# Pi-Star-Lab/RESCO

Measured on AMD Instinct MI355X. Metric: env-steps/sec, higher is better.
Workload: dtype f32; 1 GPU; ingolstadt21 x 4096 lock-step envs per GPU (BASELINE config 3), fixed demand from the map's rou.xml, on-device seeded random policy, Krauss sigma 0.5 + speedFactor dev 0.1; tls_expiry=1, map=ingolstadt21, envs_per_gpu=4096, pipes=2, ticks_per_env_step=10, block_threads=512, lds_bytes_per_env=40896, parallelism=env-batch split x1, no collective on the data path

## Files before the change

### resco_amd/csrc/resco_step.h

```cpp
#pragma once
#include "resco_tables.h"

struct State {
    char *base;
    size_t nc;
    int32_t *trip_log;
    int32_t *env;
    int32_t *tls;
    long long *stats;
    uint16_t *dep_next;
    uint32_t *mail;
    RS_HD float *pos() const { return (float *)base; }
    RS_HD float *speed() const { return RS_G((float *)(base + 4 * nc)); }
    RS_HD float *accel() const { return RS_G((float *)(base + 8 * nc)); }
    RS_HD float *tloss() const { return RS_G((float *)(base + 12 * nc)); }
    RS_HD float *sf() const { return RS_G((float *)(base + 16 * nc)); }
    RS_HD uint32_t *coop(int par) const { return RS_G((uint32_t *)(base + (par ? 43 : 20) * nc)); }
    RS_HD uint32_t *cooplead(int par) const { return RS_G((uint32_t *)(base + (par ? 47 : 24) * nc)); }
    RS_HD uint16_t *lane() const { return RS_G((uint16_t *)(base + 28 * nc)); }
    RS_HD uint16_t *trip() const { return RS_G((uint16_t *)(base + 30 * nc)); }
    RS_HD uint16_t *cursor() const { return RS_G((uint16_t *)(base + 32 * nc)); }
    RS_HD uint16_t *swait() const { return RS_G((uint16_t *)(base + 34 * nc)); }
    RS_HD uint16_t *rwait() const { return RS_G((uint16_t *)(base + 36 * nc)); }
    RS_HD uint16_t *depart() const { return RS_G((uint16_t *)(base + 38 * nc)); }
// ... 100 lines not shown
    uint8_t fl;
    uint16_t sfq;
};
#define FL_H 1
#define FL_MH 2
#define FL_LC 4
#define FL_MH1 8
RS_DEV int fl_mh(int t) { return (t & 1) ? FL_MH1 : FL_MH; }
#define LCT_LEFT 16
#define LCT_RIGHT 32
#define LCT_SWAP_LEFT 64
#define LCT_SWAP_RIGHT 128
struct __attribute__((aligned(8))) Aux {
    uint16_t lane, rq, nlink;
    uint16_t swait;
};
template <class Tp> struct LPtr {
    uint32_t off;
    RS_MEM Tp &operator[](int i) const { return ((Tp *)(RS_SMEM + off))[i]; }
    RS_MEM operator Tp *() const { return (Tp *)(RS_SMEM + off); }
};
struct Lds {
    LPtr<Node> node;
    LPtr<Aux> aux;
    LPtr<float> vnx, vtp;
    LPtr<uint16_t> grid;
    uint32_t gstride;
    LPtr<int32_t> arr;
    LPtr<uint16_t> dep, dep_t;
    LPtr<uint32_t> alive, alive0, insm;
    LPtr<uint32_t> mailw;
    LPtr<int32_t> agg_q, agg_a, agg_w, agg_m, agg_n;
    LPtr<uint32_t> agg_s;
    LPtr<int32_t> sig_arr, sig_dep;
    LPtr<int32_t> phase, left, nextp;
    LPtr<uint8_t> tstate;
    LPtr<int32_t> sc;
    LPtr<uint16_t> ls_h, ls_lc, ls_mh;
    uint32_t lcap;
    float cell_inv;
};
#define SC_T 0
#define SC_NINS 1
#define SC_HW 2
#define SC_NACT 3
#define SC_HWNEW 4
#define SC_ROOM 5
#define SC_HWOUT 6
#define SC_NH 7
#define SC_NLC 8
#define SC_NMH 9
#define SC_CHUNK_P 11
#define SC_CHUNK_M 12
#define SC_STATS 13
#ifndef RS_LIST_CHUNK
#define RS_LIST_CHUNK 64
#endif
#ifndef RS_H_CHUNK
#define RS_H_CHUNK RS_LIST_CHUNK
#endif

RS_CARVE size_t align16(size_t x) { return (x + 15) & ~(size_t)15; }
RS_CARVE int lds_list_cap(int C) {
#ifdef RS_LIST_CAP
    (void)C;
    return RS_LIST_CAP;
#else
    return ((C / 4 + 63) / 64) * 64;
#endif
}
RS_CARVE size_t lds_carve(Lds *L, int C, int n_cells, int n_arr, int n_dep, int n_obs, int S, int n_vt, int tls_maxl) {
    size_t o = 0;
#define CARVE(field, bytes) { if (L) L->field.off = (uint32_t)o; o += align16(bytes); }
    CARVE(node, (size_t)C * 16) CARVE(aux, (size_t)C * 8) CARVE(vnx, (size_t)C * 4)
    CARVE(sc, (size_t)(SC_STATS + ST_N) * 4)
    CARVE(alive, (size_t)((C + 31) / 32) * 4) CARVE(alive0, (size_t)((C + 31) / 32) * 4)
    {
        const int cap = lds_list_cap(C);
        if (L) L->lcap = (uint32_t)cap;
        CARVE(ls_h, (size_t)cap * 2) CARVE(ls_lc, (size_t)cap * 2) CARVE(ls_mh, (size_t)cap * 2)
    }
    const uint32_t grid_off = (uint32_t)o;
    const size_t grid_bytes = align16((size_t)((n_cells + 8 + 7) & ~7) * 2);
    if (L) L->gstride = (uint32_t)((n_cells + 8 + 7) & ~7);
    CARVE(grid, (size_t)((n_cells + 8 + 7) & ~7) * 2)
    CARVE(insm, (size_t)((n_dep + 31) / 32) * 4)
    CARVE(mailw, (size_t)((C + 31) / 32) * 4)
    CARVE(vtp, (size_t)n_vt * VT_COLS * 4)
    CARVE(phase, (size_t)S * 4) CARVE(left, (size_t)S * 4) CARVE(nextp, (size_t)S * 4)
    CARVE(sig_arr, (size_t)S * 4) CARVE(sig_dep, (size_t)S * 4)
    CARVE(tstate, (size_t)S * tls_maxl)
    CARVE(arr, (size_t)n_arr * 4) CARVE(dep, (size_t)n_dep * 2) CARVE(dep_t, (size_t)n_dep * 2)
    {
        const size_t ab = align16((size_t)n_obs * 4);
        uint32_t p = grid_off;
        if (6 * ab > grid_bytes) {
            p = (uint32_t)(align16((size_t)C * 16) + align16((size_t)C * 8));
            if (6 * ab > align16((size_t)C * 4)) { p = (uint32_t)o; o += 6 * ab; }
        }
        if (L) {
            L->agg_q.off = p; L->agg_a.off = p + (uint32_t)ab; L->agg_w.off = p + (uint32_t)(2 * ab);
            L->agg_m.off = p + (uint32_t)(3 * ab); L->agg_s.off = p + (uint32_t)(4 * ab); L->agg_n.off = p + (uint32_t)(5 * ab);
        }
    }
#undef CARVE
    return o;
}
// ... 265 lines not shown
    return f.slot;
}

template <class LT> RS_DEV int tls_state(const KTab &T, const LT &L, int tls, int pos) {
    if (tls == 0xFF) return TLS_G;
    return L.tstate[tls * T.tls_maxl + pos];
}
RS_DEV uint16_t cache_link(const KTab &T, const LaneRec &LR, int lane, int rq, int trip) {
    if (LR.link_cnt == 0) return NLINK_NONE;
    if (LR.flags & LF_INTERNAL) { const int l = LR.link_start; return (uint16_t)(l | (T.links()[l].arr_idx >= 0 ? NLINK_ARR : 0)); }
    return T.next_link()[((size_t)rq * T.kmax + (lane - (int)LR.edge_lane0)) * 2 + (trip & 1)];
}
template <class LT> RS_DEV bool foe_blocked(const KTab &T, const LT &L, const Grid &grid, const LinkRec &K) {
    for (int i = K.foe_start; i < K.foe_start + K.foe_cnt; ++i) {
        const FoeRec F = T.foes()[i];
        if (F.tls != 0xFF && tls_state(T, L, F.tls, F.tls_pos) == TLS_R) continue;
        if (F.arr_idx >= 0 && L.arr[F.arr_idx] < RM_FOE_GAP_Q) return true;
        if (F.via1_cell0 != 0xFFFF && cells_have_mover(grid, F.via1_cell0, F.via1_nc)) return true;
        if (F.via2_cell0 != 0xFFFF && cells_have_mover(grid, F.via2_cell0, F.via2_nc)) return true;
    }
    return false;
}
template <class LT> RS_DEV void tls_refresh(const KTab &T, const LT &L, const KParams &P, int s, int ph) {
    const int w = T.tls_maxl >> 2;
    const uint32_t *src = (const uint32_t *)((P.fixed_program ? T.cold.fix8 + T.cold.fix_state_off[s] : T.cold.tls8 + T.cold.tls_state_off[s]) + ph * T.tls_maxl);
    uint32_t *dst = (uint32_t *)((uint8_t *)L.tstate + s * T.tls_maxl);
    uint32_t v[8];
#pragma unroll
    for (int i = 0; i < 8; ++i) v[i] = src[i < w ? i : 0];
#pragma unroll
    for (int i = 0; i < 8; ++i) if (i < w) dst[i] = v[i];
#pragma unroll 1
    for (int i = 8; i < w; ++i) dst[i] = src[i];
}
template <class LT> RS_DEV void set_phase(const KTab &T, const LT &L, const KParams &P, int s, int ph) {
    if (ph < 0 || ph >= T.cold.tls_nphase[s]) return;
    L.phase[s] = ph;
    L.left[s] = P.tls_expiry ? T.cold.tls_dur[T.cold.tls_dur_off[s] + ph] : RM_TLS_HOLD_TICKS;
    tls_refresh(T, L, P, s, ph);
}
template <class LT> RS_DEV void tls_begin_of_tick(const KTab &T, const LT &L, const KParams &P, int s, int tick) {
    if (P.do_fsm && !P.fixed_program && tick == T.yellow_length) set_phase(T, L, P, s, L.nextp[s]);
    int left = L.left[s];
    if (left == 0) {
        const int32_t *dur = P.fixed_program ? T.cold.fix_dur + T.cold.fix_dur_off[s] : T.cold.tls_dur + T.cold.tls_dur_off[s];
        const int Pn = P.fixed_program ? T.cold.fix_nphase[s] : T.cold.tls_nphase[s];
        const int ph = (L.phase[s] + 1) % Pn;
        left = dur[ph];
        L.phase[s] = ph;
        tls_refresh(T, L, P, s, ph);
    }
    L.left[s] = left - 1;
}
struct ContRow { float c[4]; const float *cn; };
RS_DEV ContRow cont_row(const KTab &T, int rq) {
    ContRow R;
    R.cn = T.route_cont() + (size_t)rq * T.kmax;
    for (int j = 0; j < 4; ++j) R.c[j] = j < T.kmax ? R.cn[j] : 0.0f;
    return R;
}
RS_DEV float cont_of(const ContRow &R, int j) {
    return j == 0 ? R.c[0] : (j == 1 ? R.c[1] : (j == 2 ? R.c[2] : (j == 3 ? R.c[3] : R.cn[j])));
}
#define OCC_NONE (Grid{(uint16_t *)0, 0u})
#define OCC_FULL (Grid{(uint16_t *)1, 0u})
RS_DEV bool cont_notbest(float c) { return rs_float_as_int(c) < 0; }
RS_DEV float cont_len(float c) { return rs_int_as_float(rs_float_as_int(c) & 0x7FFFFFFF); }
RS_DEV int strategic_dir(const ContRow &R, int kk, int n, float x, float v, int extra, float &rem, const Grid &grid, int cell0, int nc, float occ_unit) {
    const float mine = cont_of(R, kk);
    rem = cont_len(mine) - x;
#ifdef RS_EMU_CHECK_MAIL
    { float best = 0.0f; for (int j = 0; j < n; ++j) { const float c = cont_len(cont_of(R, j)); if (c > best) best = c; }
      for (int j = 0; j < n; ++j) RS_ASSERT(cont_notbest(cont_of(R, j)) == !(cont_len(cont_of(R, j)) >= best - RM_CONT_EPS)) }
#endif
    if (!cont_notbest(mine)) return 0;
    int dl = 1000, dr = 1000;
    for (int j = kk + 1; j < n; ++j) if (!cont_notbest(cont_of(R, j))) { dl = j - kk; break; }
    for (int j = kk - 1; j >= 0; --j) if (!cont_notbest(cont_of(R, j))) { dr = kk - j; break; }
    const int dir = (dr <= dl) ? -1 : +1;
    if (grid.c == (uint16_t *)1) return dir;
    const int off = (dr <= dl ? dr : dl) + extra;
    const float la = (v > RM_LOOK_MIN_SPEED ? v : RM_LOOK_MIN_SPEED) * RM_LOOK_TIME + RM_LOOK_BASE;
    int cnt = 0;
    if (grid.c != (uint16_t *)0) cnt = cells_count(grid, cell0 + ((dr <= dl) ? -dr : dl) * nc, nc);
    if (rem - (float)cnt * occ_unit >= la * (float)off) return 0;
    return dir;
}
RS_DEV uint32_t link_reg_word(const KTab &T, int nlk) { return ((const uint32_t *)&T.links()[nlk & 0x7FFF])[2]; }
template <class LT> RS_DEV void register_approach_w(const KTab &T, const LT &L, uint32_t kw, float v, float pos, float lane_len, int vt) {
    const int st = tls_state(T, L, (int)((kw >> 16) & 0xFFu), (int)(kw >> 24));
    if (st == TLS_R) return;
    const float dist = lane_len - pos;
    if (st == TLS_Y && dist >= d_brake_gap(v, L.vtp[vt * VT_COLS + VT_DECEL])) return;
    const float ta = RS_DIV(dist, v > 1.0f ? v : 1.0f);
    const int q = ta * 10.0f >= 65000.0f ? 65000 : (int)(ta * 10.0f);
    rs_atomic_min(&L.arr[(int16_t)(kw & 0xFFFFu)], q);
}
template <class LT> RS_DEV void register_approach(const KTab &T, const LT &L, int nlk, float v, float pos, float lane_len, int vt) {
    if (!(nlk & NLINK_ARR)) return;
    if (v <= RM_HALT_SPEED) return;
    register_approach_w(T, L, link_reg_word(T, nlk), v, pos, lane_len, vt);
}
template <class LT> RS_DEV void follow_neighbour(const KTab &T, const LT &L, uint32_t key, bool clamp_gap, const LaneRec &LR, int lane, float x, float v,
                             float b, float tau, float mingap, float &vsafe) {
    const int X = (int)(key & 0xFFFFu), kx = (int)(key >> 16);
    if ((int)L.node[X].trip != kx) return;
    const int lx = L.aux[X].lane;
    if (lx == (int)LANE_NONE || (LR.flags & LF_INTERNAL)) return;
    const int l0 = LR.edge_lane0, n = LR.flags >> 2;
    if (lx < l0 || lx >= l0 + n) return;
    const float *vo = L.vtp + L.node[X].vt * VT_COLS;
    const float px = L.node[X].pos, backx = px - vo[VT_LENGTH];
    if (clamp_gap ? !(px >= x) : !(backx >= x)) return;
    float g = backx - x - mingap;
    if (clamp_gap && g < 0.0f) g = 0.0f;
    float vs = d_follow_speed(g, L.node[X].speed, b, vo[VT_DECEL], tau);
    float vc = v - b; if (vc < 0.0f) vc = 0.0f;
    if (vs < vc) vs = vc;
    if (vs < vsafe) vsafe = vs;
    (void)lane;
}

template <class LT> RS_DEV void mail_flag_set(const LT &L, int s, int par) { rs_atomic_or((uint32_t *)((Node *)L.node + s) + 3, SFQ_MAIL(par) << 16); }
template <class LT> RS_DEV void mail_flag_clear(const LT &L, int s, int par) { rs_atomic_and((uint32_t *)((Node *)L.node + s) + 3, ~(SFQ_MAIL(par) << 16)); }
template <class LT, class LP> RS_DEV void list_push(const LT &L, const LP &list, int counter, int s);
template <class LT> RS_DEV void flag_mover(const LT &L, int s, int t, int lct = 0) {
    uint32_t *w = (uint32_t *)((Node *)L.node + s) + 3;
    const uint32_t bit = (uint32_t)fl_mh(t) << 8;
    if (!(rs_atomic_fetch_or(w, bit | ((uint32_t)lct << 8)) & bit)) list_push(L, L.ls_mh, SC_NMH + (t & 1), s);
}
template <class LT, class LP> RS_DEV void list_push(const LT &L, const LP &list, int counter, int s) {
    const int i = rs_wave_ticket(&L.sc[counter]);
    if (i < (int)L.lcap) list[i] = (uint16_t)s;
}
RS_DEV float plan_vfree(const float *vt, float v, float lane_vmax, float sf) {
    float vfree = v + vt[VT_ACCEL];
    const float vl = lane_vmax * sf;
    if (vl < vfree) vfree = vl;
    if (vt[VT_MAXSPEED] < vfree) vfree = vt[VT_MAXSPEED];
    return vfree;
}
RS_DEV float plan_look(const float *vt, float vfree) { return d_brake_gap(vfree, vt[VT_DECEL]) + vfree * vt[VT_TAU] + vt[VT_MINGAP] + 1.0f; }
RS_DEV bool looks_beyond(const float *vt, float v, float x, float lane_len, float lane_vmax, float sf) {
    return lane_len - x < plan_look(vt, plan_vfree(vt, v, lane_vmax, sf));
}
RS_DEV bool may_change_lanes_row(const ContRow &R, const LaneRec &LR, int lane, int k, float x, float v, int t) {
    const int n = LR.flags >> 2;
    if ((LR.flags & LF_INTERNAL) || n < 2) return false;
    const int kk = lane - (int)LR.edge_lane0;
    float rem;
    if (strategic_dir(R, kk, n, x, v, 0, rem, OCC_FULL, 0, 0, 0.0f) != 0) return true;
    if ((((uint32_t)t >> 1) + (uint32_t)k) & 3u) return false;
    const int tk = kk + ((t & 1) ? -1 : +1);
    return tk >= 0 && tk < n && strategic_dir(R, tk, n, x, v, RM_SG_EXTRA_LANES, rem, OCC_NONE, 0, 0, 0.0f) == 0;
}
RS_DEV bool may_change_lanes(const KTab &T, int rq, uint32_t nb, const LaneRec &LR, int lane, int k, float x, float v, int t) {
    const int n = LR.flags >> 2;
    if ((LR.flags & LF_INTERNAL) || n < 2) return false;
    const int kk = lane - (int)LR.edge_lane0;
    bool r;
    if ((nb >> kk) & 1u) r = true;
    else if ((((uint32_t)t >> 1) + (uint32_t)k) & 3u) r = false;
    else {
        const int tk = kk + ((t & 1) ? -1 : +1);
        if (tk < 0 || tk >= n) r = false;
        else if (!((nb >> tk) & 1u)) r = true;
        else { float rem; r = strategic_dir(cont_row(T, rq), tk, n, x, v, RM_SG_EXTRA_LANES, rem, OCC_NONE, 0, 0, 0.0f) == 0; }
    }
#ifdef RS_EMU_CHECK_MAIL
    RS_ASSERT(r == may_change_lanes_row(cont_row(T, rq), LR, lane, k, x, v, t))
#endif
    return r;
}
template <class LT> RS_DEV int classify(const KTab &T, const LT &L, int s, const float *vt, float v, float x, const LaneRec &LR, int lane, int rq, uint32_t nb, int k, float sf, int t) {
    int fl = 0;
    if (looks_beyond(vt, v, x, LR.len, LR.vmax, sf)) { fl |= FL_H; list_push(L, L.ls_h, SC_NH, s); }
    if (may_change_lanes(T, rq, nb, LR, lane, k, x, v, t)) { fl |= FL_LC; list_push(L, L.ls_lc, SC_NLC, s); }
    return fl;
}

template <bool LONG, class LT> RS_DEV void phase_plan(const KTab &T, const LT &L, const Grid &grid, const State &G, size_t eo, const KParams &P, int genv, int t, int s) {
    RS_SEC_BEGIN
    const Aux ax = L.aux[s];
    const int lane = ax.lane;
    if (lane == (int)LANE_NONE) return;
    const Node me = L.node[s];
    const int k = me.trip;
    const float *vt = L.vtp + me.vt * VT_COLS;
    const float a = vt[VT_ACCEL], b = vt[VT_DECEL], tau = vt[VT_TAU], mingap = vt[VT_MINGAP];
    const float v = me.speed, x = me.pos;
    const float sf = sf_of(me.sfq);
    const LaneRec LR0 = T.lanes()[lane];
    LaneRec LR = LR0;
    float vsafe = RM_BIGF;
    float tgap = 0.0f, tvl = 0.0f, tbl = b;
    bool have = false;
    if (LONG) RS_SEC(7)
    const float vfree = plan_vfree(vt, v, LR.vmax, sf);
    const float look = plan_look(vt, vfree);
    const Found ld = leader_found(L, grid, LR.cell0, lane_cells(L, LR), x, k, s, look + T.maxlen);
    const int lead = ld.slot;
    if (LONG) RS_SEC(8)
    bool found = false;
    if (lead != NIL) {
        const float *vo = L.vtp + ld.vt() * VT_COLS;
        tgap = ld.pos() - vo[VT_LENGTH] - x - mingap;
        tvl = ld.speed(); tbl = vo[VT_DECEL];
        have = true; found = true;
    }
    if (me.sfq & SFQ_MAIL((t + 1) & 1)) {
        const int q = (t + 1) & 1;
        const uint32_t c1 = G.coop(q)[eo + s], c2 = G.cooplead(q)[eo + s];
        if (c1 != COOP_NONE) { G.coop(q)[eo + s] = COOP_NONE; follow_neighbour(T, L, c1, false, LR, lane, x, v, b, tau, mingap, vsafe); }
        if (c2 != COOP_NONE) { G.cooplead(q)[eo + s] = COOP_NONE; follow_neighbour(T, L, c2, true, LR, lane, x, v, b, tau, mingap, vsafe); }
        mail_flag_clear(L, s, q);
    }
#ifdef RS_EMU_CHECK_MAIL
    else { RS_ASSERT(G.coop((t + 1) & 1)[eo + s] == COOP_NONE && G.cooplead((t + 1) & 1)[eo + s] == COOP_NONE) }
#endif
    if (LONG) RS_SEC(9)
    float seen = LR.len - x;
    RS_ASSERT(LONG || found || !(seen < look))
    if (LONG && !found && seen < look) {
        int rq = ax.rq;
        int link = (int)(ax.nlink & 0x7FFF);
        int cur_lane = lane;
        const float bgv = d_brake_gap(v, b);
        for (int hop = 0; hop < RM_MAX_HOPS; ++hop) {
            const bool cur_int = (LR.flags & LF_INTERNAL) != 0;
            if (hop > 0) link = (int)(cache_link(T, LR, cur_lane, rq, k) & 0x7FFF);
            bool stop_here = false;
            LinkRec K;
            if (link == NLINK_NONE) {
                if (!cur_int && T.rsteps()[rq].next_edge == 0xFFFF) break;
                stop_here = true;
            } else {
                K = T.links()[link];
                const int st = tls_state(T, L, K.tls, K.tls_pos);
                if (K.tls != 0xFF && (st == TLS_R || st == TLS_Y) && seen >= bgv) stop_here = true;
                if (!stop_here && !(K.flags & KF_CONT) && ((K.flags & KF_MINOR) || (K.tls != 0xFF && st == TLS_g))) {
                    if (seen > RM_VIS_DIST) stop_here = true;
                    else if (K.foe_cnt > 0 && foe_blocked(T, L, grid, K)) stop_here = true;
                }
            }
            if (stop_here) {
                const float g = seen - RM_STOP_OFFSET;
                tgap = g > 0.0f ? g : 0.0f; tvl = 0.0f; tbl = b;
                have = true;
                break;
            }
            LR = K.dest;
            cur_lane = K.to_lane;
            {
                const float vnl = LR.vmax * sf;
                if (vnl < vfree) {
                    const float vs = d_free_speed(seen, vnl, b);
                    if (vs < vsafe) vsafe = vs;
                }
            }
            const Found od = rearmost_within(L, grid, LR.cell0, lane_cells(L, LR), look - seen + T.maxlen);
            if (od.slot != NIL) {
                const float *vo = L.vtp + od.vt() * VT_COLS;
                tgap = seen + od.pos() - vo[VT_LENGTH] - mingap;
                tvl = od.speed(); tbl = vo[VT_DECEL];
                have = true;
                break;
            }
            if (!cur_int) rq += 1;
            seen += LR.len;
            if (!(seen < look)) break;
        }
    }
    if (LONG) RS_SEC(10)
    if (have) {
        const float vs = d_follow_speed(tgap, tvl, b, tbl, tau);
        if (vs < vsafe) vsafe = vs;
    }
    float vmin_n = v - b; if (vmin_n < 0.0f) vmin_n = 0.0f;
    float vmin_e = v - vt[VT_EMERGENCY]; if (vmin_e < 0.0f) vmin_e = 0.0f;
    const float lo = vsafe > vmin_e ? vsafe : vmin_e;
    const float vmin = vmin_n < lo ? vmin_n : lo;
    float vmax = vfree < vsafe ? vfree : vsafe;
    if (vmax < vmin) vmax = vmin;
    const float sigma = P.sigma >= 0.0f ? P.sigma : vt[VT_SIGMA];
    float vd = vmax;
    if (sigma > 0.0f) {
        const float r = d_u01(d_hash(P.seed, (uint32_t)genv, (uint32_t)k, (uint32_t)t, 0u));
        if (vd < a) vd -= sigma * vd * r; else vd -= sigma * a * r;
        if (vd < 0.0f) vd = 0.0f;
    }
    const float vnext = vd > vmin ? vd : vmin;
    L.vnx[s] = vnext;
#ifdef RS_EMU_DEBUG
    if (s == rs_dbg_slot && (t == rs_dbg_t || rs_dbg_t < 0))
        printf("plan t %d slot %d lane %d x %.3f v %.3f lead %d have %d tgap %.3f tvl %.3f vsafe %.3f vfree %.3f vnext %.3f nlink %x\n", t, s, lane, x, v, lead,
               (int)have, tgap, tvl, vsafe, vfree, vnext, ax.nlink);
#endif
    if (LONG) RS_SEC(3)
    if (x + vnext > LR0.len) flag_mover(L, s, t);
    if (LONG) RS_SEC(15)
    (void)LR;
}

template <bool LONG, class LT> RS_DEV void phase_move(const KTab &T, const LT &L, const Grid &gnew, const State &G, const KParams &P, int env, size_t eo,
                       int t, bool last_tick, bool more, int s, int &active, int &halted, int &top) {
    const Aux ax = L.aux[s];
    const Node me = L.node[s];
    const int k = me.trip;
    int lane = ax.lane;
#ifdef RS_EMU_DEBUG
    {
        static int moved_at[65536];
        if (moved_at[s] == t + 1) { printf("slot %d moved twice in tick %d: fl %x lane %d trip %d\n", s, t, me.fl, lane, k); fflush(stdout); abort(); }
        moved_at[s] = t + 1;
    }
#endif
    LaneRec LR = T.lanes()[lane];
    uint32_t nb = T.notbest()[ax.rq];
// ... 30 lines not shown
    } else swn = 0;
    if (vref > 0.0f && vn < vref) { tl += RS_DIV(vref - vn, vref); G.tloss()[eo + s] = tl; }
    float x = me.pos + vn;
    bool arrived = false;
    if (LONG) for (int it = 0; it < 16; ++it) {
        if (!(x > LR.len)) break;
        const bool li = (LR.flags & LF_INTERNAL) != 0;
        if (link == NLINK_NONE) {
            if (!li && T.rsteps()[rq].next_edge == 0xFFFF) arrived = true; else x = LR.len;
            break;
        }
        x -= LR.len;
        if (!li) rq += 1;
        {
            const LinkRec Km = T.links()[link];
            lane = Km.to_lane;
            LR = Km.dest;
        }
        nlink = cache_link(T, LR, lane, rq, k);
        link = (int)(nlink & 0x7FFF);
        relink = true;
    }
    if (LONG && arrived) {
        Aux na = ax; na.lane = LANE_NONE; na.swait = 0;
        L.aux[s] = na;
        L.node[s].trip = TRIP_NONE; L.node[s].fl = (uint8_t)(me.fl & fl_mh(t));
        rs_atomic_and(&L.alive[s >> 5], ~(1u << (s & 31)));
        {
            const int ow = G.owner()[eo + s];
            if (ow != (int)OWNER_NONE) rs_atomic_add(&L.sig_dep[ow], 1);
        }
        G.owner()[eo + s] = OWNER_NONE; G.rwait()[eo + s] = 0;
        rs_atomic_add(&L.sc[SC_NACT], -1);
        rs_atomic_add(&L.sc[SC_STATS + ST_ARRIVED], 1);
        rs_atomic_add(&L.sc[SC_STATS + ST_DURATION], t + 1 - (int)G.depart()[eo + s]);
        rs_atomic_add(&L.sc[SC_STATS + ST_TLOSS], (int)(tl * 1024.0f + 0.5f));
        if (G.trip_log) {
            int32_t *r = G.trip_log + ((size_t)env * T.n_trips + k) * 4;
            r[0] = (int)G.depart()[eo + s]; r[1] = t + 1; r[2] = (int)(tl * 1024.0f + 0.5f); r[3] = (int)G.wtot()[eo + s];
        }
        return;
    }
    active += 1;
    if (s + 1 > top) top = s + 1;
    Aux na = ax;
    na.lane = (uint16_t)lane; na.rq = (uint16_t)rq; na.swait = (uint16_t)swn;
    if (LONG && relink) na.nlink = nlink;
    L.aux[s] = na;
    Node nn = me;
    nn.pos = x; nn.speed = vn; nn.fl = (uint8_t)(me.fl & fl_mh(t));
    nn.nxt = grid_push(gnew, LR.cell0 + cell_of(L, x, lane_cells(L, LR)), s, vn > RM_HALT_SPEED);
    if (more) {
        if (LONG && relink) { nb = T.notbest()[rq]; if (na.nlink & NLINK_ARR) kw = link_reg_word(T, na.nlink); }
        nn.fl |= classify(T, L, s, L.vtp + me.vt * VT_COLS, vn, x, LR, lane, rq, nb, k, sfv, t + 1);
        L.node[s] = nn;
        if ((na.nlink & NLINK_ARR) && vn > RM_HALT_SPEED) register_approach_w(T, L, kw, vn, x, LR.len, me.vt);
    } else L.node[s] = nn;
    (void)P;
}

template <class LT> RS_DEV int overlapping(const LT &L, const Grid &grid, int cell0, int ncell, float pos, int k, int self, float len_self) {
    const int lead = leader_within(L, grid, cell0, ncell, pos, k, self, RM_NB_WINDOW);
    if (lead != NIL && L.node[lead].pos - L.vtp[L.node[lead].vt * VT_COLS + VT_LENGTH] - pos < 0.0f) return lead;
    const int foll = follower_within(L, grid, cell0, ncell, pos, k, self, RM_NB_WINDOW);
    if (foll != NIL && pos - len_self - L.node[foll].pos < 0.0f) return foll;
    return NIL;
}

template <class LT> RS_DEV int phase_lc_decide(const KTab &T, const LT &L, const Grid &grid, const State &G, size_t eo, int t, int s, const Aux &ax, const Node &me) {
    const int lane = ax.lane;
    const LaneRec LR = T.lanes()[lane];
    const ContRow R = cont_row(T, ax.rq);
    const int my_wait = (int)ax.swait;
    const int n = LR.flags >> 2;
    if ((LR.flags & LF_INTERNAL) || n < 2) return 0;
    const int dir_allowed = (t & 1) ? -1 : +1;
    const int l0 = LR.edge_lane0, kk = lane - l0;
    const int k = me.trip;
    const float *vt = L.vtp + me.vt * VT_COLS;
    const float x = me.pos, v = me.speed;
    const int nc = lane_cells(L, LR);
    int want = 0, dir = dir_allowed;
    float rem;
    const int sdir = strategic_dir(R, kk, n, x, v, 0, rem, grid, LR.cell0, nc, T.occ_unit);
    if (sdir != 0) { dir = sdir; want = 2; }
    int code = 0;
    const int tk = kk + dir;
    if (tk >= 0 && tk < n) {
        const int tcell0 = (int)LR.cell0 + dir * nc;
        int lead_t = NIL, foll_t = NIL;
        bool have_t = false;
        if (!want && !((((uint32_t)t >> 1) + (uint32_t)k) & 3u)) {
            float rem_t;
            if (strategic_dir(R, tk, n, x, v, RM_SG_EXTRA_LANES, rem_t, grid, tcell0, nc, T.occ_unit) == 0) {
                const int lead_c = leader_within(L, grid, LR.cell0, nc, x, k, s, RM_NB_WINDOW);
                if (lead_c != NIL) {
                    lead_t = leader_within(L, grid, tcell0, nc, x, k, s, RM_NB_WINDOW);
                    have_t = true;
                    const float gcur = L.node[lead_c].pos - L.vtp[L.node[lead_c].vt * VT_COLS + VT_LENGTH] - x;
                    float gtgt = RM_BIGF;
                    if (lead_t != NIL) gtgt = L.node[lead_t].pos - L.vtp[L.node[lead_t].vt * VT_COLS + VT_LENGTH] - x;
                    if (gcur < v * 3.0f + 15.0f && gtgt > gcur + RM_SG_ADVANTAGE) want = 1;
                }
            }
        }
        if (want) {
            if (!have_t) lead_t = leader_within(L, grid, tcell0, nc, x, k, s, RM_NB_WINDOW);
// ... 60 lines not shown

template <class LT> RS_DEV int nth_free_slot(const LT &L, int C, int r) {
#pragma unroll 1
    for (int w = 0; w < (C + 31) / 32; ++w) {
        uint32_t fr = ~L.alive0[w];
        if (w == (C - 1) / 32 && (C & 31)) fr &= (1u << (C & 31)) - 1u;
        const int c = rs_popc(fr);
        if (r >= c) { r -= c; continue; }
#pragma unroll 1
        for (int j = 0; j < r; ++j) fr &= fr - 1u;
        return w * 32 + rs_ffs(fr) - 1;
    }
    return -1;
}

template <class LT> RS_DEV void lc_decide_and_flag(const KTab &T, const LT &L, const Grid &grid, const State &G, size_t eo, int t, int s) {
    const Aux ax = L.aux[s];
    if (ax.lane == LANE_NONE) return;
    const int code = phase_lc_decide(T, L, grid, G, eo, t, s, ax, L.node[s]);
    if (code) flag_mover(L, s, t, code);
}
struct ExecInline {};

template <int CAP, class Exec, class LT>
RS_DEV void rs_step_body_on(Exec &ex, const LT &L, const KTab &T, const State &G, const Out &O, const KParams &P,
                            const int32_t *actions, int env) {
    const int B = ex.B;
    const int C = CAP ? CAP : T.capacity, S = T.n_signals, NO = T.n_obs;
    const int genv = P.env_base + env;
    const size_t eo = (size_t)env * C;
    const int n_ticks = P.n_ticks;

    uint16_t *const grid0 = L.grid;

    ex.phase(0, [&](int tid) {
        if (tid < SC_STATS + ST_N) L.sc[tid] = tid < 4 ? G.env[env * 4 + tid] : 0;
        for (int i = tid; i < T.n_vtypes * VT_COLS; i += B) L.vtp[i] = T.cold.vtype_params[i];
        for (int i = tid; i < (int)(L.gstride >> 1); i += B) ((uint32_t *)grid0)[i] = 0x07FF07FFu;
        for (int i = tid; i < T.n_arr; i += B) L.arr[i] = ARR_NONE;
        for (int i = tid; i < (C + 31) / 32; i += B) { L.alive[i] = 0u; L.mailw[i] = 0u; }
        for (int i = tid; i < (T.n_dep + 31) / 32; i += B) L.insm[i] = 0u;
        for (int i = tid; i < T.n_dep; i += B) {
            const int k = G.dep_next[(size_t)env * T.n_dep + i];
            L.dep[i] = (uint16_t)k;
            L.dep_t[i] = k == (int)TRIP_NONE ? (uint16_t)0xFFFF : (uint16_t)T.cold.trip_depart[k];
        }
        for (int i = tid; i < S; i += B) {
            const int ph = G.tls[(env * S + i) * TLS_W + 0];
            L.phase[i] = ph;
            L.left[i] = G.tls[(env * S + i) * TLS_W + 1];
            L.nextp[i] = G.tls[(env * S + i) * TLS_W + 2];
            L.sig_arr[i] = 0; L.sig_dep[i] = G.tls[(env * S + i) * TLS_W + 3];
            tls_refresh(T, L, P, i, ph);
        }
    });
    ex.phase(1, [&](int tid) {
        const int hw0 = L.sc[SC_HW];
        for (int s = tid; s < C; s += B) {
            uint16_t ln = LANE_NONE, tr = TRIP_NONE;
            if (s < hw0) { ln = G.lane()[eo + s]; tr = G.trip()[eo + s]; }
            Aux ax; ax.lane = ln; ax.rq = 0; ax.nlink = NLINK_NONE; ax.swait = 0;
            if (ln == LANE_NONE) { L.aux[s] = ax; L.node[s].trip = TRIP_NONE; continue; }
            const float sp = G.speed()[eo + s], x = G.pos()[eo + s];
            const int rq = (int)T.routes()[T.trip_route()[tr]].start + (int)G.cursor()[eo + s];
            const LaneRec LR0 = T.lanes()[ln];
            ax.rq = (uint16_t)rq;
            ax.nlink = cache_link(T, LR0, ln, rq, tr);
            ax.swait = G.swait()[eo + s];
            L.aux[s] = ax;
            Node nn; nn.pos = x; nn.speed = sp; nn.trip = tr; nn.vt = T.trip_vtype()[tr];
            nn.fl = 0; nn.sfq = (uint16_t)speed_factor_q(P, genv, tr, L.vtp + nn.vt * VT_COLS);
            if ((G.mail[(size_t)env * ((C + 31) / 32) + (s >> 5)] >> (s & 31)) & 1u) nn.sfq |= (uint16_t)SFQ_MAIL((L.sc[SC_T] + 1) & 1);
            nn.nxt = grid_push(Grid{grid0, 0u}, LR0.cell0 + cell_of(L, x, lane_cells(L, LR0)), s, sp > RM_HALT_SPEED);
            if (n_ticks > 0) nn.fl = (uint8_t)classify(T, L, s, L.vtp + nn.vt * VT_COLS, sp, x, LR0, ln, rq, T.notbest()[rq], tr, sf_of(nn.sfq), L.sc[SC_T]);
            L.node[s] = nn;
            rs_atomic_or(&L.alive[s >> 5], 1u << (s & 31));
        }
        for (int s = B - 1 - tid; s < S; s += B) {
            if (P.do_fsm && !P.fixed_program) {
                const int a = actions[env * S + s], cur = L.phase[s], Gn = T.cold.tls_ngreen[s];
                if (a < 0 || a >= T.cold.tls_nphase[s]) L.nextp[s] = cur;
                else {
                    L.nextp[s] = a;
                    if (cur != a && cur < Gn && a < Gn) {
                        const int y = T.cold.tls_yellow[T.cold.tls_yel_off[s] + cur * Gn + a];
                        if (y >= 0) set_phase(T, L, P, s, y);
                    }
                }
            }
            if (n_ticks > 0) tls_begin_of_tick(T, L, P, s, 0);
        }
    });
    if (n_ticks > 0) ex.phase(2, [&](int tid) {
        const int hw = L.sc[SC_HW];
        for (int s = tid; s < hw; s += B) {
            const Aux ax = L.aux[s];
            if (ax.lane == LANE_NONE) continue;
            const Node me = L.node[s];
            register_approach(T, L, ax.nlink, me.speed, me.pos, T.lanes()[ax.lane].len, me.vt);
        }
    });

    int cur = 0;
    for (int tick = 0; tick < n_ticks; ++tick) {
        const int t = L.sc[SC_T], hw = L.sc[cur ? SC_HWNEW : SC_HW];
        const Grid gold{grid0, cur ? CELL_TAG : 0u}, gnew{grid0, cur ? 0u : CELL_TAG};
        const bool more = tick + 1 < n_ticks;
        const int lcap = (int)L.lcap;
        const int nwv = B >> 6;
        ex.phase(4, [&](int tid) {
            const int wv = ex.wave_of(tid), ln = tid & 63;
            const int nh = L.sc[SC_NH], nlc = L.sc[SC_NLC];
            const unsigned long long r0 = ex.role_begin();
            int role = 0;
            if (nh > lcap || nlc > lcap) {
                for (int pass = 0; pass < 2; ++pass)
                    for (int w = tid; w < hw; w += B) {
                        if (pass && !(L.node[w].fl & FL_LC)) continue;
                        if (pass) lc_decide_and_flag(T, L, gold, G, eo, t, w);
                        else phase_plan<true>(T, L, gold, G, eo, P, genv, t, w);
                    }
            } else {
                const int hch = (nh + RS_H_CHUNK - 1) / RS_H_CHUNK, lch = (nlc + RS_LIST_CHUNK - 1) / RS_LIST_CHUNK;
                const int total = hch + lch + ((hw + 63) >> 6);
                for (int it = 0;; ++it) {
                    const int c = ex.next_chunk(&L.sc[SC_CHUNK_P], wv, it, nwv);
                    if (c >= total) break;
                    if (c < hch) {
                        role = 1;
                        const int w = c * RS_H_CHUNK + ln;
                        if (ln < RS_H_CHUNK && w < nh) phase_plan<true>(T, L, gold, G, eo, P, genv, t, L.ls_h[w]);
                    } else if (c < hch + lch) {
                        role = 2;
                        const int w = (c - hch) * RS_LIST_CHUNK + ln;
                        if (ln < RS_LIST_CHUNK && w < nlc) lc_decide_and_flag(T, L, gold, G, eo, t, L.ls_lc[w]);
                    } else {
                        const int w = (c - hch - lch) * 64 + ln;
                        if (w < hw && !(L.node[w].fl & FL_H)) phase_plan<false>(T, L, gold, G, eo, P, genv, t, w);
                    }
                }
            }
            ex.role_end(role == 1 ? 7 : (role == 2 ? 8 : 9), r0);
            for (int i = tid; i < (T.n_dep + 31) / 32; i += B) L.insm[i] = 0u;
        });
        ex.phase(5, [&](int tid) {
            for (int i = tid; i < T.n_arr; i += B) L.arr[i] = ARR_NONE;
            for (int i = tid; i < (C + 31) / 32; i += B) L.alive0[i] = L.alive[i];
            int Bs = B;
            RS_OPAQUE_S(Bs)
            for (int i = tid; i < (int)(L.gstride >> 2); i += Bs) {
                unsigned long long *q = (unsigned long long *)grid0 + i;
                const unsigned long long w = *q;
                const unsigned long long st = ((w ^ grid_tag4(gold)) >> 15) & 0x0001000100010001ull;
                if (st) { const unsigned long long m = st * 0xFFFFull; *q = (w & ~m) | ((0x07FF07FF07FF07FFull | grid_tag4(gold)) & m); }
            }
            for (int d = B - 1 - tid; d < T.n_dep; d += B)
                if (phase_insert_decide(T, L, gold, t, d)) rs_atomic_or(&L.insm[d >> 5], 1u << (d & 31));
            if (more)
                for (int sg = B - 1 - tid; sg < S; sg += B) tls_begin_of_tick(T, L, P, sg, tick + 1);
            if (tid == 0) {
                L.sc[SC_T] = t + 1; L.sc[SC_STATS + ST_TICKS] += 1;
                L.sc[cur ? SC_HW : SC_HWNEW] = 0;
                L.sc[SC_ROOM] = C - L.sc[SC_NACT];
                L.sc[SC_NH] = 0; L.sc[SC_NLC] = 0;
                L.sc[SC_NMH + ((t + 1) & 1)] = 0;
                L.sc[SC_CHUNK_P] = 0; L.sc[SC_CHUNK_M] = 0;
            }
        });
        ex.phase(6, [&](int tid) {
            int active = 0, halted = 0, top = 0;
            const int wv = ex.wave_of(tid), ln = tid & 63;
            const int nmh = L.sc[SC_NMH + (t & 1)];
            int ich = 0;
            for (int i = 0; i < (T.n_dep + 31) / 32; ++i) if (L.insm[i]) ich = 1;
            const bool all = nmh > lcap;
            const int mch = all ? 0 : (nmh + RS_LIST_CHUNK - 1) / RS_LIST_CHUNK;
            const int total = mch + ich + ((hw + 63) >> 6);
            const unsigned long long r0 = ex.role_begin();
            bool list = false;
            for (int it = 0;; ++it) {
                const int c = ex.next_chunk(&L.sc[SC_CHUNK_M], wv, it, nwv);
                if (c >= total) break;
                if (c < mch) {
                    list = true;
                    const int w = c * RS_LIST_CHUNK + ln;
                    if (ln < RS_LIST_CHUNK && w < nmh) phase_move<true>(T, L, gnew, G, P, env, eo, t, !more, more, L.ls_mh[w], active, halted, top);
                } else if (c < mch + ich) {
                    for (int d = 63 - ln; d < T.n_dep; d += 64) {
                        if (!(L.insm[d >> 5] & (1u << (d & 31)))) continue;
                        int rank = rs_popc(L.insm[d >> 5] & ((1u << (d & 31)) - 1u));
                        for (int w = 0; w < (d >> 5); ++w) rank += rs_popc(L.insm[w]);
                        if (rank >= L.sc[SC_ROOM]) { rs_atomic_add(&L.sc[SC_STATS + ST_CAP_BLOCKED], 1); continue; }
                        const int s = nth_free_slot(L, C, rank);
                        if (s < 0) continue;
                        const int k = L.dep[d];
                        const int v = T.trip_vtype()[k];
                        const float *vt = L.vtp + v * VT_COLS;
                        const RouteRec RR = T.routes()[T.trip_route()[k]];
                        const LaneRec LRd = T.lanes()[RR.depart_lane];
                        const int sfq = speed_factor_q(P, genv, k, vt);
                        const float sfn = sf_of(sfq);
                        Node nn; nn.pos = vt[VT_LENGTH] < RR.depart_len ? vt[VT_LENGTH] : RR.depart_len;
                        nn.speed = 0.0f; nn.trip = (uint16_t)k; nn.vt = (uint8_t)v; nn.fl = 0; nn.sfq = (uint16_t)sfq;
                        nn.nxt = grid_push(gnew, LRd.cell0 + cell_of(L, nn.pos, lane_cells(L, LRd)), s, false);
                        if (more) nn.fl = (uint8_t)classify(T, L, s, vt, 0.0f, nn.pos, LRd, RR.depart_lane, (int)RR.start, T.notbest()[RR.start], k, sfn, t + 1);
                        L.node[s] = nn;
                        Aux na; na.lane = RR.depart_lane; na.rq = (uint16_t)RR.start; na.swait = 0;
                        na.nlink = cache_link(T, LRd, RR.depart_lane, (int)RR.start, k);
                        L.aux[s] = na;
                        G.sf()[eo + s] = sfn; G.tloss()[eo + s] = 0.0f; G.cooplead(0)[eo + s] = COOP_NONE; G.cooplead(1)[eo + s] = COOP_NONE; G.coop(0)[eo + s] = COOP_NONE; G.coop(1)[eo + s] = COOP_NONE;
                        G.rwait()[eo + s] = 0; G.owner()[eo + s] = OWNER_NONE; G.depart()[eo + s] = (uint16_t)(t + 1); G.accel()[eo + s] = 0.0f; G.wtot()[eo + s] = 0;
                        {
                            const int k2 = T.cold.trip_next[k];
                            L.dep[d] = (uint16_t)k2;
                            L.dep_t[d] = k2 == (int)TRIP_NONE ? (uint16_t)0xFFFF : (uint16_t)T.cold.trip_depart[k2];
                        }
                        rs_atomic_or(&L.alive[s >> 5], 1u << (s & 31));
                        rs_atomic_add(&L.sc[SC_NACT], 1);
                        rs_atomic_add(&L.sc[SC_NINS], 1);
                        rs_atomic_add(&L.sc[SC_STATS + ST_INSERTED], 1);
                        rs_atomic_add(&L.sc[SC_STATS + ST_DEPDELAY], t - T.cold.trip_depart[k]);
                        if (s + 1 > top) top = s + 1;
                    }
                } else {
                    const int w = (c - mch - ich) * 64 + ln;
                    if (w < hw && (L.alive0[w >> 5] & (1u << (w & 31)))) {
                        if (all) phase_move<true>(T, L, gnew, G, P, env, eo, t, !more, more, w, active, halted, top);
                        else if (!(L.node[w].fl & fl_mh(t))) phase_move<false>(T, L, gnew, G, P, env, eo, t, !more, more, w, active, halted, top);
                    }
                }
            }
            ex.role_end(list ? 10 : 3, r0);
            rs_wave_add(&L.sc[SC_STATS + ST_ACTIVE_TICKS], active);
            rs_wave_add(&L.sc[SC_STATS + ST_WAITING], halted);
            rs_wave_max(&L.sc[cur ? SC_HW : SC_HWNEW], top);
            ex.role_end(15, r0);
        });
        cur ^= 1;
    }
    const int hw_end = L.sc[cur ? SC_HWNEW : SC_HW];

    const bool obs = P.do_observe != 0;
    if (obs) ex.phase(11, [&](int tid) {
        for (int i = tid; i < NO; i += B) { L.agg_q[i] = 0; L.agg_a[i] = 0; L.agg_w[i] = 0; L.agg_m[i] = 0; L.agg_s[i] = 0; L.agg_n[i] = 0; }
    });
    ex.phase(12, [&](int tid) {
        const int hw0 = G.env[env * 4 + 2];
        const int top = hw_end > hw0 ? hw_end : hw0;
        int hi = 0;
        for (int s = tid; s < top; s += B) {
            const int lane = L.aux[s].lane;
            G.lane()[eo + s] = (uint16_t)lane; G.trip()[eo + s] = L.node[s].trip;
            if (lane == (int)LANE_NONE) continue;
            hi = s + 1;
            if (L.node[s].sfq & SFQ_MAIL((L.sc[SC_T] + 1) & 1)) rs_atomic_or(&L.mailw[s >> 5], 1u << (s & 31));
            const int rq = L.aux[s].rq;
            G.pos()[eo + s] = L.node[s].pos; G.speed()[eo + s] = L.node[s].speed; G.swait()[eo + s] = L.aux[s].swait;
            G.cursor()[eo + s] = (uint16_t)(rq - (int)T.routes()[T.trip_route()[L.node[s].trip]].start);
            if (!obs) continue;
            const int prev_owner = G.owner()[eo + s];
            const LaneRec LR = T.lanes()[lane];
            const int oi = T.cold.lane_obs[lane];
// ... 49 lines not shown
            if (l < T.cold.sig_obs_start[sg + 1] - o0) {
                const int oi = o0 + l;
                if (c == 0) nrm = l == L.phase[sg] ? 1.0f : 0.0f;
                else if (c == 1) nrm = (float)L.agg_a[oi] / 28.0f;
                else if (c == 2) nrm = (float)L.agg_w[oi] / 28.0f;
                else if (c == 3) nrm = (float)L.agg_q[oi] / 28.0f;
                else nrm = (float)L.agg_s[oi] * (1.0f / 65536.0f) / 20.0f / 28.0f;
            }
            O.drq_f16()[(size_t)env * S * T.lmax * 5 + i] = rs_f2h(nrm);
        }
        if (om & (OUT_MPLIGHT | OUT_WAVE | OUT_MPLIGHT_FULL)) for (int i = tid; i < S * 12; i += B) {
            const int sg = i / 12, m = i - sg * 12;
            int q = 0, wv = 0, tw = 0, ap = 0;
            float last_speed = 0.0f;
            for (int j = T.cold.mv_in_start[i]; j < T.cold.mv_in_start[i + 1]; ++j) {
                const int oi = T.cold.mv_in_idx[j];
                q += L.agg_q[oi]; wv += L.agg_q[oi] + L.agg_a[oi]; tw += L.agg_w[oi]; ap += L.agg_a[oi];
                last_speed = (float)L.agg_s[oi] * (1.0f / 65536.0f);
            }
            for (int j = T.cold.mv_out_start[i]; j < T.cold.mv_out_start[i + 1]; ++j) q -= L.agg_q[T.cold.mv_out_idx[j]];
            const size_t so = (size_t)env * S + sg;
            if (om & OUT_MPLIGHT) O.mplight()[so * 13 + 1 + m] = q;
            if (om & OUT_WAVE) O.wave()[so * 12 + m] = wv;
            if (om & OUT_MPLIGHT_FULL) {
                float *mf = O.mplight_full() + so * 49 + 1 + m * 4;
                mf[0] = (float)q; mf[1] = (float)tw / 28.0f; mf[2] = last_speed; mf[3] = (float)ap / 28.0f;
            }
        }
        for (int sg = tid; sg < S; sg += B) {
            const int ph = L.phase[sg];
            if (obs) {
                const int o0 = T.cold.sig_obs_start[sg], o1 = T.cold.sig_obs_start[sg + 1];
                int tw = 0, tq = 0, mq = 0;
                for (int oi = o0; oi < o1; ++oi) { tw += L.agg_w[oi]; const int qq = L.agg_q[oi]; tq += qq; if (qq > mq) mq = qq; }
                const size_t so = (size_t)env * S + sg;
                O.phase()[so] = ph; O.queue_sum()[so] = tq; O.queue_max()[so] = mq;
                O.wait()[so] = -(float)tw;
                const float wn = -(float)tw / 224.0f;
                O.wait_norm()[so] = wn < -4.0f ? -4.0f : (wn > 4.0f ? 4.0f : wn);
                int pr = tq;
                for (int i = T.cold.pr_out_start[sg]; i < T.cold.pr_out_start[sg + 1]; ++i) pr -= L.agg_q[T.cold.pr_out_idx[i]];
                O.pressure()[so] = -pr;
                if (om & OUT_MPLIGHT) O.mplight()[so * 13] = ph;
                if (om & OUT_MPLIGHT_FULL) O.mplight_full()[so * 49] = (float)ph;
                O.arrivals()[so] = L.sig_arr[sg]; O.departures()[so] = L.sig_dep[sg];
            }
            G.tls[(env * S + sg) * TLS_W + 0] = ph;
            G.tls[(env * S + sg) * TLS_W + 1] = L.left[sg];
            G.tls[(env * S + sg) * TLS_W + 2] = L.nextp[sg];
            G.tls[(env * S + sg) * TLS_W + 3] = obs ? 0 : L.sig_dep[sg];
        }
        for (int i = tid; i < T.n_dep; i += B) G.dep_next[(size_t)env * T.n_dep + i] = L.dep[i];
        for (int i = tid; i < (C + 31) / 32; i += B) G.mail[(size_t)env * ((C + 31) / 32) + i] = L.mailw[i];
    });
    ex.phase(14, [&](int tid) {
        if (tid == 0) {
            G.env[env * 4 + 0] = L.sc[SC_T]; G.env[env * 4 + 1] = L.sc[SC_NINS]; G.env[env * 4 + 3] = L.sc[SC_NACT];
            G.env[env * 4 + 2] = L.sc[SC_HWOUT];
        }
        if (tid < ST_N) {
            long long *st = G.stats + (size_t)env * ST_N;
            if (tid == ST_ACTIVE) st[tid] = L.sc[SC_NACT];
            else if (tid == ST_PENDING) {
                const int t = L.sc[SC_T];
                const int hz = t - 1 <= T.horizon ? t - 1 : T.horizon;
                st[tid] = (t >= 1 ? T.cold.trips_cum[hz] : 0) - L.sc[SC_NINS];
            } else st[tid] += L.sc[SC_STATS + tid];
        }
    });
}

template <int CAP, class Exec>
RS_DEV void rs_step_body(Exec &ex, const Lds &L, const KTab &T, const State &G, const Out &O, const KParams &P,
                         const int32_t *actions, int env) {
    if constexpr (CAP != 0) {
        const LdsFix<CAP> Lf(L);
        rs_step_body_on<CAP>(ex, Lf, T, G, O, P, actions, env);
    } else rs_step_body_on<CAP>(ex, L, T, G, O, P, actions, env);
}
```

Baseline: 3.895 million env-steps/s.

## Split halo planning into single-hop and multi-hop lists; merge setup phases

The classifier now computes the look-ahead distance once, caches it per vehicle, and sorts beyond-lane vehicles into a single-hop list or a multi-hop list. The multi-hop list fills from the top of the shared buffer. Single-hop vehicles run a specialised planner that stops after one link, which reduces divergence and loop work in the planning phase. Signal preparation and approach registration move into the existing init phases, and the final two output phases are merged, removing several block barriers. Risks include the extra LDS field vnx (it must exist in the layout) and the two lists sharing one buffer's capacity.

```diff
diff --git a/resco_amd/csrc/resco_step.h b/resco_amd/csrc/resco_step.h
--- a/resco_amd/csrc/resco_step.h
+++ b/resco_amd/csrc/resco_step.h
@@ -176,7 +176,8 @@
 #define SC_NMH 9
 #define SC_CHUNK_P 11
 #define SC_CHUNK_M 12
-#define SC_STATS 13
+#define SC_NH2 13
+#define SC_STATS 14
 #ifndef RS_LIST_CHUNK
 #define RS_LIST_CHUNK 64
 #endif
@@ -548,6 +549,20 @@
     }
     L.left[s] = left - 1;
 }
+template <class LT> RS_DEV void signal_prep(const KTab &T, const LT &L, const KParams &P, const int32_t *actions, int env, int s, int n_ticks) {
+    if (P.do_fsm && !P.fixed_program) {
+        const int a = actions[env * T.n_signals + s], cur = L.phase[s], Gn = T.cold.tls_ngreen[s];
+        if (a < 0 || a >= T.cold.tls_nphase[s]) L.nextp[s] = cur;
+        else {
+            L.nextp[s] = a;
+            if (cur != a && cur < Gn && a < Gn) {
+                const int y = T.cold.tls_yellow[T.cold.tls_yel_off[s] + cur * Gn + a];
+                if (y >= 0) set_phase(T, L, P, s, y);
+            }
+        }
+    }
+    if (n_ticks > 0) tls_begin_of_tick(T, L, P, s, 0);
+}
 struct ContRow { float c[4]; const float *cn; };
 RS_DEV ContRow cont_row(const KTab &T, int rq) {
     ContRow R;
@@ -637,9 +652,6 @@
     return vfree;
 }
 RS_DEV float plan_look(const float *vt, float vfree) { return d_brake_gap(vfree, vt[VT_DECEL]) + vfree * vt[VT_TAU] + vt[VT_MINGAP] + 1.0f; }
-RS_DEV bool looks_beyond(const float *vt, float v, float x, float lane_len, float lane_vmax, float sf) {
-    return lane_len - x < plan_look(vt, plan_vfree(vt, v, lane_vmax, sf));
-}
 RS_DEV bool may_change_lanes_row(const ContRow &R, const LaneRec &LR, int lane, int k, float x, float v, int t) {
     const int n = LR.flags >> 2;
     if ((LR.flags & LF_INTERNAL) || n < 2) return false;
@@ -668,14 +680,28 @@
 #endif
     return r;
 }
-template <class LT> RS_DEV int classify(const KTab &T, const LT &L, int s, const float *vt, float v, float x, const LaneRec &LR, int lane, int rq, uint32_t nb, int k, float sf, int t) {
+template <class LT> RS_DEV int classify(const KTab &T, const LT &L, int s, const float *vt, float v, float x, const LaneRec &LR, int lane, int rq, uint32_t nb, int k, float sf, int t, int nlink) {
     int fl = 0;
-    if (looks_beyond(vt, v, x, LR.len, LR.vmax, sf)) { fl |= FL_H; list_push(L, L.ls_h, SC_NH, s); }
+    const float look = plan_look(vt, plan_vfree(vt, v, LR.vmax, sf));
+    L.vnx[s] = look;
+    const float seen = LR.len - x;
+    if (seen < look) {
+        fl |= FL_H;
+        const int link = nlink & 0x7FFF;
+        bool multi = false;
+        if (link != NLINK_NONE) multi = seen + T.links()[link].dest.len < look;
+        if (multi) {
+            const int i = rs_wave_ticket(&L.sc[SC_NH2]);
+            if (i < (int)L.lcap) L.ls_h[(int)L.lcap - 1 - i] = (uint16_t)s;
+        } else list_push(L, L.ls_h, SC_NH, s);
+    }
     if (may_change_lanes(T, rq, nb, LR, lane, k, x, v, t)) { fl |= FL_LC; list_push(L, L.ls_lc, SC_NLC, s); }
     return fl;
 }
 
-template <bool LONG, class LT> RS_DEV void phase_plan(const KTab &T, const LT &L, const Grid &grid, const State &G, size_t eo, const KParams &P, int genv, int t, int s) {
+template <int MODE, class LT> RS_DEV void phase_plan(const KTab &T, const LT &L, const Grid &grid, const State &G, size_t eo, const KParams &P, int genv, int t, int s) {
+    constexpr bool LONG = MODE != 0;
+    constexpr int HOPS = MODE == 1 ? 1 : RM_MAX_HOPS;
     RS_SEC_BEGIN
     const Aux ax = L.aux[s];
     const int lane = ax.lane;
@@ -693,7 +719,8 @@
     bool have = false;
     if (LONG) RS_SEC(7)
     const float vfree = plan_vfree(vt, v, LR.vmax, sf);
-    const float look = plan_look(vt, vfree);
+    const float look = L.vnx[s];
+    RS_ASSERT(look == plan_look(vt, vfree))
     const Found ld = leader_found(L, grid, LR.cell0, lane_cells(L, LR), x, k, s, look + T.maxlen);
     const int lead = ld.slot;
     if (LONG) RS_SEC(8)
@@ -722,7 +749,7 @@
         int link = (int)(ax.nlink & 0x7FFF);
         int cur_lane = lane;
         const float bgv = d_brake_gap(v, b);
-        for (int hop = 0; hop < RM_MAX_HOPS; ++hop) {
+        for (int hop = 0; hop < HOPS; ++hop) {
             const bool cur_int = (LR.flags & LF_INTERNAL) != 0;
             if (hop > 0) link = (int)(cache_link(T, LR, cur_lane, rq, k) & 0x7FFF);
             bool stop_here = false;
@@ -760,6 +787,10 @@
                 tgap = seen + od.pos() - vo[VT_LENGTH] - mingap;
                 tvl = od.speed(); tbl = vo[VT_DECEL];
                 have = true;
+                break;
+            }
+            if (MODE == 1) {
+                RS_ASSERT(!(seen + LR.len < look))
                 break;
             }
             if (!cur_int) rq += 1;
@@ -896,7 +927,7 @@
     nn.nxt = grid_push(gnew, LR.cell0 + cell_of(L, x, lane_cells(L, LR)), s, vn > RM_HALT_SPEED);
     if (more) {
         if (LONG && relink) { nb = T.notbest()[rq]; if (na.nlink & NLINK_ARR) kw = link_reg_word(T, na.nlink); }
-        nn.fl |= classify(T, L, s, L.vtp + me.vt * VT_COLS, vn, x, LR, lane, rq, nb, k, sfv, t + 1);
+        nn.fl |= classify(T, L, s, L.vtp + me.vt * VT_COLS, vn, x, LR, lane, rq, nb, k, sfv, t + 1, na.nlink);
         L.node[s] = nn;
         if ((na.nlink & NLINK_ARR) && vn > RM_HALT_SPEED) register_approach_w(T, L, kw, vn, x, LR.len, me.vt);
     } else L.node[s] = nn;
@@ -1063,6 +1094,7 @@
             L.nextp[i] = G.tls[(env * S + i) * TLS_W + 2];
             L.sig_arr[i] = 0; L.sig_dep[i] = G.tls[(env * S + i) * TLS_W + 3];
             tls_refresh(T, L, P, i, ph);
+            signal_prep(T, L, P, actions, env, i, n_ticks);
         }
     });
     ex.phase(1, [&](int tid) {
@@ -1083,32 +1115,10 @@
             nn.fl = 0; nn.sfq = (uint16_t)speed_factor_q(P, genv, tr, L.vtp + nn.vt * VT_COLS);
             if ((G.mail[(size_t)env * ((C + 31) / 32) + (s >> 5)] >> (s & 31)) & 1u) nn.sfq |= (uint16_t)SFQ_MAIL((L.sc[SC_T] + 1) & 1);
             nn.nxt = grid_push(Grid{grid0, 0u}, LR0.cell0 + cell_of(L, x, lane_cells(L, LR0)), s, sp > RM_HALT_SPEED);
-            if (n_ticks > 0) nn.fl = (uint8_t)classify(T, L, s, L.vtp + nn.vt * VT_COLS, sp, x, LR0, ln, rq, T.notbest()[rq], tr, sf_of(nn.sfq), L.sc[SC_T]);
+            if (n_ticks > 0) nn.fl = (uint8_t)classify(T, L, s, L.vtp + nn.vt * VT_COLS, sp, x, LR0, ln, rq, T.notbest()[rq], tr, sf_of(nn.sfq), L.sc[SC_T], ax.nlink);
             L.node[s] = nn;
             rs_atomic_or(&L.alive[s >> 5], 1u << (s & 31));
-        }
-        for (int s = B - 1 - tid; s < S; s += B) {
-            if (P.do_fsm && !P.fixed_program) {
-                const int a = actions[env * S + s], cur = L.phase[s], Gn = T.cold.tls_ngreen[s];
-                if (a < 0 || a >= T.cold.tls_nphase[s]) L.nextp[s] = cur;
-                else {
-                    L.nextp[s] = a;
-                    if (cur != a && cur < Gn && a < Gn) {
-                        const int y = T.cold.tls_yellow[T.cold.tls_yel_off[s] + cur * Gn + a];
-                        if (y >= 0) set_phase(T, L, P, s, y);
-                    }
-                }
-            }
-            if (n_ticks > 0) tls_begin_of_tick(T, L, P, s, 0);
-        }
-    });
-    if (n_ticks > 0) ex.phase(2, [&](int tid) {
-        const int hw = L.sc[SC_HW];
-        for (int s = tid; s < hw; s += B) {
-            const Aux ax = L.aux[s];
-            if (ax.lane == LANE_NONE) continue;
-            const Node me = L.node[s];
-            register_approach(T, L, ax.nlink, me.speed, me.pos, T.lanes()[ax.lane].len, me.vt);
+            if (n_ticks > 0) register_approach(T, L, ax.nlink, sp, x, LR0.len, nn.vt);
         }
     });
 
@@ -1121,37 +1131,42 @@
         const int nwv = B >> 6;
         ex.phase(4, [&](int tid) {
             const int wv = ex.wave_of(tid), ln = tid & 63;
-            const int nh = L.sc[SC_NH], nlc = L.sc[SC_NLC];
+            const int nh = L.sc[SC_NH], nh2 = L.sc[SC_NH2], nlc = L.sc[SC_NLC];
             const unsigned long long r0 = ex.role_begin();
             int role = 0;
-            if (nh > lcap || nlc > lcap) {
+            if (nh + nh2 > lcap || nlc > lcap) {
                 for (int pass = 0; pass < 2; ++pass)
                     for (int w = tid; w < hw; w += B) {
                         if (pass && !(L.node[w].fl & FL_LC)) continue;
                         if (pass) lc_decide_and_flag(T, L, gold, G, eo, t, w);
-                        else phase_plan<true>(T, L, gold, G, eo, P, genv, t, w);
+                        else phase_plan<2>(T, L, gold, G, eo, P, genv, t, w);
                     }
             } else {
-                const int hch = (nh + RS_H_CHUNK - 1) / RS_H_CHUNK, lch = (nlc + RS_LIST_CHUNK - 1) / RS_LIST_CHUNK;
+                const int h2ch = (nh2 + RS_H_CHUNK - 1) / RS_H_CHUNK, hch = h2ch + (nh + RS_H_CHUNK - 1) / RS_H_CHUNK;
+                const int lch = (nlc + RS_LIST_CHUNK - 1) / RS_LIST_CHUNK;
                 const int total = hch + lch + ((hw + 63) >> 6);
                 for (int it = 0;; ++it) {
                     const int c = ex.next_chunk(&L.sc[SC_CHUNK_P], wv, it, nwv);
                     if (c >= total) break;
-                    if (c < hch) {
-                        role = 1;
+                    if (c < h2ch) {
+                        if (!role) role = 1;
                         const int w = c * RS_H_CHUNK + ln;
-                        if (ln < RS_H_CHUNK && w < nh) phase_plan<true>(T, L, gold, G, eo, P, genv, t, L.ls_h[w]);
+                        if (ln < RS_H_CHUNK && w < nh2) phase_plan<2>(T, L, gold, G, eo, P, genv, t, L.ls_h[lcap - 1 - w]);
+                    } else if (c < hch) {
+                        if (!role) role = 3;
+                        const int w = (c - h2ch) * RS_H_CHUNK + ln;
+                        if (ln < RS_H_CHUNK && w < nh) phase_plan<1>(T, L, gold, G, eo, P, genv, t, L.ls_h[w]);
                     } else if (c < hch + lch) {
-                        role = 2;
+                        if (!role) role = 2;
                         const int w = (c - hch) * RS_LIST_CHUNK + ln;
                         if (ln < RS_LIST_CHUNK && w < nlc) lc_decide_and_flag(T, L, gold, G, eo, t, L.ls_lc[w]);
                     } else {
                         const int w = (c - hch - lch) * 64 + ln;
-                        if (w < hw && !(L.node[w].fl & FL_H)) phase_plan<false>(T, L, gold, G, eo, P, genv, t, w);
+                        if (w < hw && !(L.node[w].fl & FL_H)) phase_plan<0>(T, L, gold, G, eo, P, genv, t, w);
                     }
                 }
             }
-            ex.role_end(role == 1 ? 7 : (role == 2 ? 8 : 9), r0);
+            ex.role_end(role == 1 ? 7 : (role == 3 ? 14 : (role == 2 ? 8 : 9)), r0);
             for (int i = tid; i < (T.n_dep + 31) / 32; i += B) L.insm[i] = 0u;
         });
         ex.phase(5, [&](int tid) {
@@ -1173,7 +1188,7 @@
                 L.sc[SC_T] = t + 1; L.sc[SC_STATS + ST_TICKS] += 1;
                 L.sc[cur ? SC_HW : SC_HWNEW] = 0;
                 L.sc[SC_ROOM] = C - L.sc[SC_NACT];
-                L.sc[SC_NH] = 0; L.sc[SC_NLC] = 0;
+                L.sc[SC_NH] = 0; L.sc[SC_NH2] = 0; L.sc[SC_NLC] = 0;
                 L.sc[SC_NMH + ((t + 1) & 1)] = 0;
                 L.sc[SC_CHUNK_P] = 0; L.sc[SC_CHUNK_M] = 0;
             }
@@ -1214,11 +1229,11 @@
                         Node nn; nn.pos = vt[VT_LENGTH] < RR.depart_len ? vt[VT_LENGTH] : RR.depart_len;
                         nn.speed = 0.0f; nn.trip = (uint16_t)k; nn.vt = (uint8_t)v; nn.fl = 0; nn.sfq = (uint16_t)sfq;
                         nn.nxt = grid_push(gnew, LRd.cell0 + cell_of(L, nn.pos, lane_cells(L, LRd)), s, false);
-                        if (more) nn.fl = (uint8_t)classify(T, L, s, vt, 0.0f, nn.pos, LRd, RR.depart_lane, (int)RR.start, T.notbest()[RR.start], k, sfn, t + 1);
-                        L.node[s] = nn;
                         Aux na; na.lane = RR.depart_lane; na.rq = (uint16_t)RR.start; na.swait = 0;
                         na.nlink = cache_link(T, LRd, RR.depart_lane, (int)RR.start, k);
                         L.aux[s] = na;
+                        if (more) nn.fl = (uint8_t)classify(T, L, s, vt, 0.0f, nn.pos, LRd, RR.depart_lane, (int)RR.start, T.notbest()[RR.start], k, sfn, t + 1, na.nlink);
+                        L.node[s] = nn;
                         G.sf()[eo + s] = sfn; G.tloss()[eo + s] = 0.0f; G.cooplead(0)[eo + s] = COOP_NONE; G.cooplead(1)[eo + s] = COOP_NONE; G.coop(0)[eo + s] = COOP_NONE; G.coop(1)[eo + s] = COOP_NONE;
                         G.rwait()[eo + s] = 0; G.owner()[eo + s] = OWNER_NONE; G.depart()[eo + s] = (uint16_t)(t + 1); G.accel()[eo + s] = 0.0f; G.wtot()[eo + s] = 0;
                         {
@@ -1374,8 +1389,6 @@
         }
         for (int i = tid; i < T.n_dep; i += B) G.dep_next[(size_t)env * T.n_dep + i] = L.dep[i];
         for (int i = tid; i < (C + 31) / 32; i += B) G.mail[(size_t)env * ((C + 31) / 32) + i] = L.mailw[i];
-    });
-    ex.phase(14, [&](int tid) {
         if (tid == 0) {
             G.env[env * 4 + 0] = L.sc[SC_T]; G.env[env * 4 + 1] = L.sc[SC_NINS]; G.env[env * 4 + 3] = L.sc[SC_NACT];
             G.env[env * 4 + 2] = L.sc[SC_HWOUT];
```

Result: no change. 3.934 million env-steps/s, median of 6 (+1.0%).
